# samedii/perceptor

Hardware: AMD Instinct MI355X
Metric: denoising steps/sec (UNet+CLIP-grad) at 512x512 batch 8 (higher is better)
Workload: dtype bf16

## Files before the change

perceptor_amd/csrc/attn.hip:

```cpp
#include "common.h"
#include "../../include/perceptor_hip.h"

namespace {

__device__ __forceinline__ int64_t tfrag(int bh, int ntb, int tb, int ks, int db, int lhi, int l31) {
  return ((((((int64_t)bh * ntb + tb) * 2 + ks) * 2 + db) * 2 + lhi) * 32 + l31) * 8;
}

__device__ __forceinline__ int64_t rfrag(int bh, int ntb, int tb, int kk, int lhi, int l31) {
  return ((((((int64_t)bh * ntb + tb) * 4 + kk) * 2 + lhi) * 32 + l31) * 8);
}

template <typename T_>
__global__ __launch_bounds__(256) void qkv_split_kernel(const u16* __restrict__ qkv, u16* __restrict__ q,
                                                        u16* __restrict__ k, u16* __restrict__ vt, int T, int Tp,
                                                        int heads, int order) {
  __shared__ u16 sv[32][72];
  const int tid = threadIdx.x, t0 = blockIdx.x * 32, bh = blockIdx.y;
  const int n = bh / heads, h = bh - n * heads;
  const int C = heads * 64;
  const int qoff = order == 0 ? h * 192 : h * 64;
  const int koff = order == 0 ? h * 192 + 64 : C + h * 64;
  const int voff = order == 0 ? h * 192 + 128 : 2 * C + h * 64;
  const int row = tid >> 3, ch = tid & 7;
// ... 162 lines not shown
                                                          int T, int Tp, int heads) {
  __shared__ u16 s[32][72];
  const int tid = threadIdx.x, t0 = blockIdx.x * 32, bh = blockIdx.y;
  const int n = bh / heads, h = bh - n * heads, C = heads * 64;
  const int row = tid >> 3, ch = tid & 7, t = t0 + row;
  uint4 val = make_uint4(0, 0, 0, 0), ov = val;
  if (t < T) {
    val = *(const uint4*)(dout + ((int64_t)n * T + t) * C + h * 64 + ch * 8);
    ov = *(const uint4*)(o + ((int64_t)n * T + t) * C + h * 64 + ch * 8);
  }
  *(uint4*)(d_o + rfrag(bh, Tp >> 5, blockIdx.x, ch >> 1, ch & 1, row)) = val;
  *(uint4*)(&s[row][ch * 8]) = val;
  float a[8], b[8], p = 0.f;
  unpack8<T_>(val, a); unpack8<T_>(ov, b);
#pragma unroll
  for (int e = 0; e < 8; ++e) p += a[e] * b[e];
  p += __shfl_xor(p, 1); p += __shfl_xor(p, 2); p += __shfl_xor(p, 4);
  if (ch == 0) delta[(int64_t)bh * Tp + t] = p;
  __syncthreads();
  const int d = tid >> 2, tc = tid & 3, fks = tc >> 1, flhi = tc & 1;
  u16 e[8];
#pragma unroll
  for (int j = 0; j < 8; ++j) e[j] = s[16 * fks + 4 * flhi + (j & 3) + 8 * (j >> 2)][d];
  *(uint4*)(d_ot + tfrag(bh, Tp >> 5, blockIdx.x, fks, d >> 5, flhi, d & 31)) =
      make_uint4(e[0] | (e[1] << 16), e[2] | (e[3] << 16), e[4] | (e[5] << 16), e[6] | (e[7] << 16));
}

template <typename T_>
__global__ __launch_bounds__(64) void vit_attn_fwd_kernel(const u16* __restrict__ q, const u16* __restrict__ k, const u16* __restrict__ vt,
                                                          u16* __restrict__ out, float* __restrict__ lse, int T, int Tp, int heads, float scale) {
  const int lane = threadIdx.x, l31 = lane & 31, lhi = lane >> 5;
  int bx, bh;
  head_xcd_remap(bx, bh);
  const int t0 = bx * 32;
  const int ntb = Tp >> 5;
  uint4 qf[4];
#pragma unroll
  for (int kk = 0; kk < 4; ++kk) qf[kk] = *(const uint4*)(q + rfrag(bh, ntb, bx, kk, lhi, l31));
  f32x16 o0, o1;
#pragma unroll
  for (int r = 0; r < 16; ++r) { o0[r] = 0.f; o1[r] = 0.f; }
  float m_run = -1e30f, l_run = 0.f;
  struct Tile { uint4 k[4], vt[2][2]; };
  auto load_tile = [&](int sb, Tile& f) {
#pragma unroll
    for (int kk = 0; kk < 4; ++kk) f.k[kk] = *(const uint4*)(k + rfrag(bh, ntb, sb, kk, lhi, l31));
#pragma unroll
    for (int ks = 0; ks < 2; ++ks)
#pragma unroll
      for (int db = 0; db < 2; ++db) f.vt[ks][db] = *(const uint4*)(vt + tfrag(bh, ntb, sb, ks, db, lhi, l31));
  };
  auto compute = [&](const Tile& f, int s0) {
    f32x16 sacc;
#pragma unroll
    for (int r = 0; r < 16; ++r) sacc[r] = 0.f;
#pragma unroll
    for (int kk = 0; kk < 4; ++kk) sacc = T_::mfma32(f.k[kk], qf[kk], sacc);
    float mx = -1e30f;
#pragma unroll
    for (int r = 0; r < 16; ++r) {
      const int s = s0 + (r & 3) + 8 * (r >> 2) + 4 * lhi;
      const float v = s < T ? sacc[r] * scale : -1e30f;
      sacc[r] = v; mx = fmaxf(mx, v);
    }
    mx = fmaxf(mx, __shfl_xor(mx, 32));
    const float m_new = fmaxf(m_run, mx), alpha = __expf(m_run - m_new);
    float rs = 0.f;
#pragma unroll
    for (int r = 0; r < 16; ++r) { const float p = __expf(sacc[r] - m_new); sacc[r] = p; rs += p; }
    rs += __shfl_xor(rs, 32);
    l_run = l_run * alpha + rs; m_run = m_new;
#pragma unroll
    for (int r = 0; r < 16; ++r) { o0[r] *= alpha; o1[r] *= alpha; }
#pragma unroll
    for (int ks = 0; ks < 2; ++ks) {
      float pf[8];
#pragma unroll
      for (int j = 0; j < 8; ++j) pf[j] = sacc[8 * ks + j];
      const uint4 pfrag = pack8<T_>(pf);
      o0 = T_::mfma32(f.vt[ks][0], pfrag, o0);
      o1 = T_::mfma32(f.vt[ks][1], pfrag, o1);
    }
  };
  Tile ta, tb_;
  load_tile(0, ta);
  for (int sb = 0; sb < ntb; sb += 2) {
    load_tile(sb + 1 < ntb ? sb + 1 : sb, tb_);
    __builtin_amdgcn_sched_barrier(0);
    compute(ta, sb * 32);
    __builtin_amdgcn_sched_barrier(0);
    if (sb + 1 < ntb) {
      load_tile(sb + 2 < ntb ? sb + 2 : sb + 1, ta);
      __builtin_amdgcn_sched_barrier(0);
      compute(tb_, (sb + 1) * 32);
      __builtin_amdgcn_sched_barrier(0);
    }
  }
  const int t = t0 + l31;
  if (lhi == 0) lse[(int64_t)bh * Tp + t] = t < T ? m_run + __logf(l_run) : 0.f;
  if (t < T) {
    const float inv = 1.f / l_run;
    const int n = bh / heads, h = bh - n * heads;
    u16* ob = out + ((int64_t)n * T + t) * (heads * 64) + h * 64 + 4 * lhi;
#pragma unroll
    for (int g = 0; g < 4; ++g) {
      *(uint2*)(ob + 8 * g) = pack4<T_>(o0[4 * g] * inv, o0[4 * g + 1] * inv, o0[4 * g + 2] * inv, o0[4 * g + 3] * inv);
      *(uint2*)(ob + 32 + 8 * g) = pack4<T_>(o1[4 * g] * inv, o1[4 * g + 1] * inv, o1[4 * g + 2] * inv, o1[4 * g + 3] * inv);
    }
  }
}

template <typename T_>
__device__ __forceinline__ void vit_attn_dq_body(const u16* __restrict__ q, const u16* __restrict__ k, const u16* __restrict__ v,
                                                 const u16* __restrict__ kt, const u16* __restrict__ d_o,
                                                 const float* __restrict__ lse, const float* __restrict__ delta,
                                                 u16* __restrict__ dqkv, int T, int Tp, int heads, float scale, int bx, int bh) {
  const int lane = threadIdx.x, l31 = lane & 31, lhi = lane >> 5;
  const int t0 = bx * 32;
  const int64_t rb = (int64_t)bh * Tp;
  uint4 qf[4], dof[4];
#pragma unroll
  for (int kk = 0; kk < 4; ++kk) {
    qf[kk] = *(const uint4*)(q + rfrag(bh, Tp >> 5, bx, kk, lhi, l31));
    dof[kk] = *(const uint4*)(d_o + rfrag(bh, Tp >> 5, bx, kk, lhi, l31));
  }
  const float my_lse = lse[rb + t0 + l31], my_delta = delta[rb + t0 + l31];
  f32x16 g0, g1;
#pragma unroll
  for (int r = 0; r < 16; ++r) { g0[r] = 0.f; g1[r] = 0.f; }
  struct Tile { uint4 k[4], v[4], kt[2][2]; };
  const int ntb = Tp >> 5;
  auto load_tile = [&](int sb, Tile& f) {
#pragma unroll
    for (int kk = 0; kk < 4; ++kk) {
      f.k[kk] = *(const uint4*)(k + rfrag(bh, ntb, sb, kk, lhi, l31));
      f.v[kk] = *(const uint4*)(v + rfrag(bh, ntb, sb, kk, lhi, l31));
    }
#pragma unroll
    for (int ks = 0; ks < 2; ++ks)
#pragma unroll
      for (int db = 0; db < 2; ++db) f.kt[ks][db] = *(const uint4*)(kt + tfrag(bh, ntb, sb, ks, db, lhi, l31));
  };
  auto compute = [&](const Tile& f, int s0) {
    f32x16 sacc, dp;
#pragma unroll
    for (int r = 0; r < 16; ++r) { sacc[r] = 0.f; dp[r] = 0.f; }
#pragma unroll
    for (int kk = 0; kk < 4; ++kk) {
      sacc = T_::mfma32(f.k[kk], qf[kk], sacc);
      dp = T_::mfma32(f.v[kk], dof[kk], dp);
    }
#pragma unroll
    for (int r = 0; r < 16; ++r) {
      const int s = s0 + (r & 3) + 8 * (r >> 2) + 4 * lhi;
      const float p = s < T ? __expf(sacc[r] * scale - my_lse) : 0.f;
      sacc[r] = p * (dp[r] - my_delta) * scale;
    }
#pragma unroll
    for (int ks = 0; ks < 2; ++ks) {
      float g[8];
#pragma unroll
      for (int j = 0; j < 8; ++j) g[j] = sacc[8 * ks + j];
      const uint4 dsf = pack8<T_>(g);
      g0 = T_::mfma32(f.kt[ks][0], dsf, g0);
      g1 = T_::mfma32(f.kt[ks][1], dsf, g1);
    }
  };
  Tile ta, tb_;
  load_tile(0, ta);
  for (int sb = 0; sb < ntb; sb += 2) {
    load_tile(sb + 1 < ntb ? sb + 1 : sb, tb_);
    __builtin_amdgcn_sched_barrier(0);
    compute(ta, sb * 32);
    __builtin_amdgcn_sched_barrier(0);
    if (sb + 1 < ntb) {
      load_tile(sb + 2 < ntb ? sb + 2 : sb + 1, ta);
      __builtin_amdgcn_sched_barrier(0);
      compute(tb_, (sb + 1) * 32);
      __builtin_amdgcn_sched_barrier(0);
    }
  }
  const int t = t0 + l31;
  if (t < T) {
    const int n = bh / heads, h = bh - n * heads, C = heads * 64;
    u16* ob = dqkv + ((int64_t)n * T + t) * 3 * C + h * 64 + 4 * lhi;
#pragma unroll
    for (int g = 0; g < 4; ++g) {
      *(uint2*)(ob + 8 * g) = pack4<T_>(g0[4 * g], g0[4 * g + 1], g0[4 * g + 2], g0[4 * g + 3]);
      *(uint2*)(ob + 32 + 8 * g) = pack4<T_>(g1[4 * g], g1[4 * g + 1], g1[4 * g + 2], g1[4 * g + 3]);
    }
  }
}

template <typename T_>
__device__ __forceinline__ void vit_attn_dkdv_body(const u16* __restrict__ q, const u16* __restrict__ k, const u16* __restrict__ v,
                                                   const u16* __restrict__ qt, const u16* __restrict__ d_o, const u16* __restrict__ d_ot,
                                                   const float* __restrict__ lse, const float* __restrict__ delta,
                                                   u16* __restrict__ dqkv, int T, int Tp, int heads, float scale, int bx, int bh) {
  const int lane = threadIdx.x, l31 = lane & 31, lhi = lane >> 5;
  const int s0 = bx * 32;
  const int64_t rb = (int64_t)bh * Tp;
  uint4 kf[4], vf[4];
#pragma unroll
  for (int kk = 0; kk < 4; ++kk) {
    kf[kk] = *(const uint4*)(k + rfrag(bh, Tp >> 5, bx, kk, lhi, l31));
    vf[kk] = *(const uint4*)(v + rfrag(bh, Tp >> 5, bx, kk, lhi, l31));
  }
  const bool key_ok = s0 + l31 < T;
  f32x16 dk0, dk1, dv0, dv1;
#pragma unroll
  for (int r = 0; r < 16; ++r) { dk0[r] = 0.f; dk1[r] = 0.f; dv0[r] = 0.f; dv1[r] = 0.f; }
  struct Tile { uint4 q[4], dO[4], dot[2][2], qt[2][2]; float ls[16], dl[16]; };
  const int ntb = Tp >> 5;
  auto load_tile = [&](int tb, Tile& f) {
#pragma unroll
    for (int kk = 0; kk < 4; ++kk) {
      f.q[kk] = *(const uint4*)(q + rfrag(bh, ntb, tb, kk, lhi, l31));
      f.dO[kk] = *(const uint4*)(d_o + rfrag(bh, ntb, tb, kk, lhi, l31));
    }
#pragma unroll
    for (int ks = 0; ks < 2; ++ks)
#pragma unroll
      for (int db = 0; db < 2; ++db) {
        const int64_t fo = tfrag(bh, ntb, tb, ks, db, lhi, l31);
        f.dot[ks][db] = *(const uint4*)(d_ot + fo); f.qt[ks][db] = *(const uint4*)(qt + fo);
      }
#pragma unroll
    for (int r = 0; r < 16; ++r) {
      const int t = tb * 32 + (r & 3) + 8 * (r >> 2) + 4 * lhi;
      f.ls[r] = lse[rb + t]; f.dl[r] = delta[rb + t];
    }
  };
  auto compute = [&](const Tile& f, int t0) {
    f32x16 sacc, dp;
#pragma unroll
    for (int r = 0; r < 16; ++r) { sacc[r] = 0.f; dp[r] = 0.f; }
#pragma unroll
    for (int kk = 0; kk < 4; ++kk) {
      sacc = T_::mfma32(f.q[kk], kf[kk], sacc);
      dp = T_::mfma32(f.dO[kk], vf[kk], dp);
    }
    float pf[16];
#pragma unroll
    for (int r = 0; r < 16; ++r) {
      const int t = t0 + (r & 3) + 8 * (r >> 2) + 4 * lhi;
      const float p = (key_ok && t < T) ? __expf(sacc[r] * scale - f.ls[r]) : 0.f;
      pf[r] = p;
      sacc[r] = p * (dp[r] - f.dl[r]) * scale;
    }
#pragma unroll
    for (int ks = 0; ks < 2; ++ks) {
      const uint4 pfrag = pack8<T_>(pf + 8 * ks);
      float g[8];
#pragma unroll
      for (int j = 0; j < 8; ++j) g[j] = sacc[8 * ks + j];
      const uint4 dsf = pack8<T_>(g);
      dv0 = T_::mfma32(f.dot[ks][0], pfrag, dv0); dk0 = T_::mfma32(f.qt[ks][0], dsf, dk0);
      dv1 = T_::mfma32(f.dot[ks][1], pfrag, dv1); dk1 = T_::mfma32(f.qt[ks][1], dsf, dk1);
    }
  };
  Tile ta, tb_;
  load_tile(0, ta);
  for (int tb = 0; tb < ntb; tb += 2) {
    load_tile(tb + 1 < ntb ? tb + 1 : tb, tb_);
    __builtin_amdgcn_sched_barrier(0);
    compute(ta, tb * 32);
    __builtin_amdgcn_sched_barrier(0);
    if (tb + 1 < ntb) {
      load_tile(tb + 2 < ntb ? tb + 2 : tb + 1, ta);
      __builtin_amdgcn_sched_barrier(0);
      compute(tb_, (tb + 1) * 32);
      __builtin_amdgcn_sched_barrier(0);
    }
  }
  const int s = s0 + l31;
  if (s < T) {
    const int n = bh / heads, h = bh - n * heads, C = heads * 64;
    u16* okp = dqkv + ((int64_t)n * T + s) * 3 * C + C + h * 64 + 4 * lhi;
    u16* ovp = okp + C;
#pragma unroll
    for (int g = 0; g < 4; ++g) {
      *(uint2*)(okp + 8 * g) = pack4<T_>(dk0[4 * g], dk0[4 * g + 1], dk0[4 * g + 2], dk0[4 * g + 3]);
      *(uint2*)(okp + 32 + 8 * g) = pack4<T_>(dk1[4 * g], dk1[4 * g + 1], dk1[4 * g + 2], dk1[4 * g + 3]);
      *(uint2*)(ovp + 8 * g) = pack4<T_>(dv0[4 * g], dv0[4 * g + 1], dv0[4 * g + 2], dv0[4 * g + 3]);
      *(uint2*)(ovp + 32 + 8 * g) = pack4<T_>(dv1[4 * g], dv1[4 * g + 1], dv1[4 * g + 2], dv1[4 * g + 3]);
    }
  }
}

template <typename T_>
__global__ __launch_bounds__(64) void vit_attn_bwd_kernel(const u16* __restrict__ q, const u16* __restrict__ k, const u16* __restrict__ v,
                                                          const u16* __restrict__ qt, const u16* __restrict__ kt,
                                                          const u16* __restrict__ d_o, const u16* __restrict__ d_ot,
                                                          const float* __restrict__ lse, const float* __restrict__ delta,
                                                          u16* __restrict__ dqkv, int T, int Tp, int heads, float scale) {
  int bx, bh;
  head_xcd_remap(bx, bh);
  if (blockIdx.z == 0) vit_attn_dkdv_body<T_>(q, k, v, qt, d_o, d_ot, lse, delta, dqkv, T, Tp, heads, scale, bx, bh);
  else vit_attn_dq_body<T_>(q, k, v, kt, d_o, lse, delta, dqkv, T, Tp, heads, scale, bx, bh);
}

}

#define VIT_BY_DTYPE(KERN, G, B, ...)                                                             \
  do {                                                                                            \
    if (dtype == PMI_DT_BF16) hipLaunchKernelGGL(KERN<BF16>, G, B, 0, (hipStream_t)s, __VA_ARGS__); \
    else hipLaunchKernelGGL(KERN<F16>, G, B, 0, (hipStream_t)s, __VA_ARGS__);                     \
  } while (0)

extern "C" int pmi_vit_attn_fwd(const void* qkv, void* ws16, float* lse, void* out, int N, int T, int heads, float scale, int dtype,
                                pmi_stream_t s) {
  if (!qkv || !ws16 || !lse || !out || N <= 0 || T <= 0 || heads <= 0) return PMI_ERR_ARG;
  const int Tp = (T + 31) / 32 * 32;
  const int64_t blk = (int64_t)N * heads * Tp * 64;
  u16* w = (u16*)ws16;
  dim3 g(Tp / 32, N * heads);
  VIT_BY_DTYPE(vit_qkv_split_kernel, g, dim3(256), (const u16*)qkv, w, w + blk, w + 2 * blk, w + 3 * blk, w + 4 * blk, w + 5 * blk, T, Tp, heads);
  PMI_CHECK_LAUNCH();
  VIT_BY_DTYPE(vit_attn_fwd_kernel, g, dim3(64), w, w + blk, w + 5 * blk, (u16*)out, lse, T, Tp, heads, scale);
  PMI_CHECK_LAUNCH();
  return PMI_OK;
}

extern "C" int pmi_vit_attn_bwd(const void* ws16, const float* lse, const void* o, const void* dout, void* ws16b, float* delta,
                                void* dqkv, int N, int T, int heads, float scale, int dtype, pmi_stream_t s) {
  if (!ws16 || !lse || !o || !dout || !ws16b || !delta || !dqkv || N <= 0 || T <= 0 || heads <= 0) return PMI_ERR_ARG;
  const int Tp = (T + 31) / 32 * 32;
  const int64_t blk = (int64_t)N * heads * Tp * 64;
  const u16* w = (const u16*)ws16;
  u16* wb = (u16*)ws16b;
  dim3 g(Tp / 32, N * heads);
  VIT_BY_DTYPE(vit_do_prep_kernel, g, dim3(256), (const u16*)dout, (const u16*)o, wb, wb + blk, delta, T, Tp, heads);
  PMI_CHECK_LAUNCH();
  dim3 g2(Tp / 32, N * heads, 2);
  VIT_BY_DTYPE(vit_attn_bwd_kernel, g2, dim3(64), w, w + blk, w + 2 * blk, w + 3 * blk, w + 4 * blk, wb, wb + blk, lse, delta, (u16*)dqkv, T, Tp,
               heads, scale);
  PMI_CHECK_LAUNCH();
  return PMI_OK;
}
```

perceptor_amd/csrc/igemm.hip:

```cpp
#include <cstdio>
#include <cstdlib>
#include "common.h"
#include "epilogue.h"
#include "../../include/perceptor_hip.h"

namespace {

constexpr int BM = 128, BN = 128, BK = 64;
constexpr int TILE_BYTES = 128 * 128;
constexpr int STAGE_BYTES = 2 * TILE_BYTES;

__device__ __forceinline__ int lds_off(int row, int chunk) { return row * 128 + ((chunk ^ ((row >> 1) & 7)) << 4); }

template <typename T, bool CONV, bool KFAST, bool PHASED = false>
__global__ __launch_bounds__(256, 2) void igemm_kernel(const pmi_igemm_args a) {
  static_assert(!PHASED || CONV, "the phased geometry is a convolution");
  __shared__ __attribute__((aligned(16))) char smem[2 * STAGE_BYTES];

  const int tid = threadIdx.x, lane = tid & 63, wid = tid >> 6;
  const int wr = wid >> 1, wc = wid & 1;
#ifdef PMI_STAMPS
#define GSTAMP(k) do { if (tid == 0 && a.reserved == 77 && a.splitk <= 1) ((long long*)a.ws)[(int64_t)blockIdx.x * 8 + (k)] = (long long)wall_clock64(); } while (0)
#else
#define GSTAMP(k) do {} while (0)
// ... 267 lines not shown
#pragma unroll
    for (int e = 0; e < 16; ++e) cs[e] = 0.f;
#pragma unroll
    for (int t = 0; t < 8; ++t) {
      const int m = m0 + wr * 64 + 8 * t + rp;
      uint4 v = *(const uint4*)(stg + (8 * t + rp) * SROW + r8 * 16);
      if (a.R || a.stats) {
        float f[8];
        unpack8<T>(v, f);
        if (a.R) {
          float r[8];
          unpack8<T>(rres[t], r);
#pragma unroll
          for (int e = 0; e < 8; ++e) f[e] += r[e];
          v = pack8<T>(f);
        }
        if (m < a.M) {
#pragma unroll
          for (int e = 0; e < 8; ++e) { cs[e] += f[e]; cs[8 + e] += f[e] * f[e]; }
        }
      }
      if (nok && m < Mr) *(uint4*)((u16*)a.D + offD + orow(m) * a.ldd + n0 + cl0) = v;
    }
    if (a.stats) {
      float b8[8], b4[4], b2[2];
      const bool h3 = lane & 8, h4 = lane & 16, h5 = lane & 32;
#pragma unroll
      for (int k = 0; k < 8; ++k) { const float mine = h3 ? cs[k + 8] : cs[k], other = h3 ? cs[k] : cs[k + 8]; b8[k] = mine + __shfl_xor(other, 8); }
#pragma unroll
      for (int k = 0; k < 4; ++k) { const float mine = h4 ? b8[k + 4] : b8[k], other = h4 ? b8[k] : b8[k + 4]; b4[k] = mine + __shfl_xor(other, 16); }
#pragma unroll
      for (int k = 0; k < 2; ++k) { const float mine = h5 ? b4[k + 2] : b4[k], other = h5 ? b4[k] : b4[k + 2]; b2[k] = mine + __shfl_xor(other, 32); }
      const int e0 = (h4 ? 4 : 0) + (h5 ? 2 : 0);
      float* const slot = stat + wr * 2 * BN;
      slot[2 * (cl0 + e0) + (h3 ? 1 : 0)] = b2[0];
      slot[2 * (cl0 + e0 + 1) + (h3 ? 1 : 0)] = b2[1];
    }
  } else {
  int64_t rrow[2];
  const float* nbp[2];
  int mrow[2];
#pragma unroll
  for (int i = 0; i < 2; ++i) {
    const int m = m0 + wr * 64 + i * 32 + l31;
    mrow[i] = m;
    rrow[i] = (int64_t)m * a.ldr;
    if (a.R && a.res_up && m < a.M) {
      const int hw = a.H * a.W;
      const int img = m / hw, rem = m - img * hw;
      const int y = rem / a.W, x = rem - y * a.W;
      rrow[i] = ((int64_t)(img * (a.H >> 1) + (y >> 1)) * (a.W >> 1) + (x >> 1)) * a.ldr;
    }
    nbp[i] = (a.nbias && m < a.M) ? a.nbias + (int64_t)(m / a.hw) * (a.ldnb ? a.ldnb : a.N) : nullptr;
  }
#pragma unroll
  for (int j = 0; j < 2; ++j) {
    float ssum[16], ssq[16];
#pragma unroll
    for (int r = 0; r < 16; ++r) { ssum[r] = 0.f; ssq[r] = 0.f; }
    float4 rv[2][4], bv[4], nbv[2][4];
#pragma unroll
    for (int g = 0; g < 4; ++g) {
      const int n = n0 + wc * 64 + j * 32 + 4 * lhi + 8 * g;
      bv[g] = make_float4(0.f, 0.f, 0.f, 0.f);
      if (a.bias && n < a.N) bv[g] = *(const float4*)(a.bias + n);
#pragma unroll
      for (int i = 0; i < 2; ++i) {
        nbv[i][g] = make_float4(0.f, 0.f, 0.f, 0.f);
        if (nbp[i] && n < a.N) nbv[i][g] = *(const float4*)(nbp[i] + n);
      }
    }
    if (a.R) {
#pragma unroll
      for (int i = 0; i < 2; ++i)
#pragma unroll
        for (int g = 0; g < 4; ++g) {
          const int n = n0 + wc * 64 + j * 32 + 4 * lhi + 8 * g;
          rv[i][g] = make_float4(0.f, 0.f, 0.f, 0.f);
          if (mrow[i] >= a.M || n >= a.N) continue;
          if (a.res_f32) {
            rv[i][g] = *(const float4*)((const float*)a.R + offR + rrow[i] + n);
          } else if (a.split_out) {
            const int po = split_off(n, a.split_out);
            const uint2 rh = *(const uint2*)((const u16*)a.R + offR + rrow[i] + po);
            const uint2 rl = *(const uint2*)((const u16*)a.R + offR + rrow[i] + po + a.split_out);
            rv[i][g].x = __builtin_bit_cast(float, rh.x); rv[i][g].y = __builtin_bit_cast(float, rh.y);
            rv[i][g].z = __builtin_bit_cast(float, rl.x); rv[i][g].w = __builtin_bit_cast(float, rl.y);
          } else {
            const uint2 r = *(const uint2*)((const u16*)a.R + offR + rrow[i] + n);
            rv[i][g].x = __builtin_bit_cast(float, r.x); rv[i][g].y = __builtin_bit_cast(float, r.y);
          }
        }
    }
#pragma unroll
    for (int i = 0; i < 2; ++i) {
      const int m = mrow[i];
      if (m >= Mr) continue;
      const int64_t mo = orow(m);
#pragma unroll
      for (int g = 0; g < 4; ++g) {
        const int n = n0 + wc * 64 + j * 32 + 4 * lhi + 8 * g;
        if (n >= a.N) continue;
        float v[4];
#pragma unroll
        for (int e = 0; e < 4; ++e) v[e] = acc[i][j][4 * g + e] * a.alpha;
        v[0] += bv[g].x + nbv[i][g].x; v[1] += bv[g].y + nbv[i][g].y; v[2] += bv[g].z + nbv[i][g].z; v[3] += bv[g].w + nbv[i][g].w;
        if (a.act != PMI_ACT_NONE) act_apply_n<4>(v, a.act);
        if (a.R) {
          if (a.res_f32) {
            v[0] += rv[i][g].x; v[1] += rv[i][g].y; v[2] += rv[i][g].z; v[3] += rv[i][g].w;
          } else {
            const uint32_t r0 = __builtin_bit_cast(uint32_t, rv[i][g].x), r1 = __builtin_bit_cast(uint32_t, rv[i][g].y);
            v[0] += T::to_f((u16)(r0 & 0xffff)); v[1] += T::to_f((u16)(r0 >> 16));
            v[2] += T::to_f((u16)(r1 & 0xffff)); v[3] += T::to_f((u16)(r1 >> 16));
            if (a.split_out) {
              const uint32_t l0 = __builtin_bit_cast(uint32_t, rv[i][g].z), l1 = __builtin_bit_cast(uint32_t, rv[i][g].w);
              v[0] += T::to_f((u16)(l0 & 0xffff)); v[1] += T::to_f((u16)(l0 >> 16));
              v[2] += T::to_f((u16)(l1 & 0xffff)); v[3] += T::to_f((u16)(l1 >> 16));
            }
          }
        }
        if (a.split_out) {
          const int64_t o = offD + (int64_t)m * a.ldd + split_off(n, a.split_out);
          const uint2 hi = pack4<T>(v[0], v[1], v[2], v[3]);
          const float l0 = v[0] - T::to_f((u16)(hi.x & 0xffff)), l1 = v[1] - T::to_f((u16)(hi.x >> 16));
          const float l2 = v[2] - T::to_f((u16)(hi.y & 0xffff)), l3 = v[3] - T::to_f((u16)(hi.y >> 16));
          *(uint2*)((u16*)a.D + o) = hi;
          *(uint2*)((u16*)a.D + o + a.split_out) = pack4<T>(l0, l1, l2, l3);
        } else {
        const int64_t o = offD + mo * a.ldd + n;
        if (a.out_f32) *(float4*)((float*)a.D + o) = make_float4(v[0], v[1], v[2], v[3]);
        else *(uint2*)((u16*)a.D + o) = pack4<T>(v[0], v[1], v[2], v[3]);
        }
#pragma unroll
        for (int e = 0; e < 4; ++e) { ssum[4 * g + e] += v[e]; ssq[4 * g + e] += v[e] * v[e]; }
      }
    }
    if (a.stats) stats_block_to_lds(ssum, ssq, stat + wr * 2 * BN, wc * 64 + j * 32, lane);
  }
  }
  if (a.stats) {
    __syncthreads();
    const int img = m0 / a.hw, prow = (m0 - img * a.hw) / BM;
    float* o = a.stats + ((int64_t)(img * a.stats_p + prow) * a.N + n0) * 2;
    for (int c = tid; c < 2 * BN; c += 256)
      if (n0 + (c >> 1) < a.N) o[c] = stat[c] + stat[2 * BN + c];
  }
#ifdef PMI_STAMPS
  __syncthreads();
  GSTAMP(3);
#endif
}

template <typename T>
__global__ __launch_bounds__(256) void splitk_reduce_kernel(const pmi_igemm_args a) {
  const int n4 = a.N >> 2;
  const int64_t total = (int64_t)a.M * n4;
  const float* ws = (const float*)a.ws;
  for (int64_t i = (int64_t)blockIdx.x * 256 + threadIdx.x; i < total; i += (int64_t)gridDim.x * 256) {
    const int m = (int)(i / n4), n = (int)(i - (int64_t)m * n4) * 4;
    float4 s = make_float4(0.f, 0.f, 0.f, 0.f);
    for (int z = 0; z < a.splitk; ++z) {
      const float4 p = *(const float4*)(ws + ((int64_t)z * a.M + m) * a.N + n);
      s.x += p.x; s.y += p.y; s.z += p.z; s.w += p.w;
    }
    float v[4] = {s.x * a.alpha, s.y * a.alpha, s.z * a.alpha, s.w * a.alpha};
    if (a.bias) { const float4 b = *(const float4*)(a.bias + n); v[0] += b.x; v[1] += b.y; v[2] += b.z; v[3] += b.w; }
    if (a.nbias) {
      const float4 b = *(const float4*)(a.nbias + (int64_t)(m / a.hw) * (a.ldnb ? a.ldnb : a.N) + n);
      v[0] += b.x; v[1] += b.y; v[2] += b.z; v[3] += b.w;
    }
    if (a.act != PMI_ACT_NONE) act_apply_n<4>(v, a.act);
    if (a.R) {
      int64_t rrow = (int64_t)m * a.ldr;
      if (a.res_up) {
        const int hw = a.H * a.W;
        const int img = m / hw, rem = m - img * hw;
        const int y = rem / a.W, x = rem - y * a.W;
        rrow = ((int64_t)(img * (a.H >> 1) + (y >> 1)) * (a.W >> 1) + (x >> 1)) * a.ldr;
      }
      if (a.res_f32) {
        const float4 r = *(const float4*)((const float*)a.R + rrow + n);
        v[0] += r.x; v[1] += r.y; v[2] += r.z; v[3] += r.w;
      } else {
        const int po = a.split_out ? split_off(n, a.split_out) : n;
        const uint2 r = *(const uint2*)((const u16*)a.R + rrow + po);
        v[0] += T::to_f((u16)(r.x & 0xffff)); v[1] += T::to_f((u16)(r.x >> 16));
        v[2] += T::to_f((u16)(r.y & 0xffff)); v[3] += T::to_f((u16)(r.y >> 16));
        if (a.split_out) {
          const uint2 l = *(const uint2*)((const u16*)a.R + rrow + po + a.split_out);
          v[0] += T::to_f((u16)(l.x & 0xffff)); v[1] += T::to_f((u16)(l.x >> 16));
          v[2] += T::to_f((u16)(l.y & 0xffff)); v[3] += T::to_f((u16)(l.y >> 16));
        }
      }
    }
    if (a.split_out) {
      const int64_t o = (int64_t)m * a.ldd + split_off(n, a.split_out);
      const uint2 hi = pack4<T>(v[0], v[1], v[2], v[3]);
      const float l0 = v[0] - T::to_f((u16)(hi.x & 0xffff)), l1 = v[1] - T::to_f((u16)(hi.x >> 16));
      const float l2 = v[2] - T::to_f((u16)(hi.y & 0xffff)), l3 = v[3] - T::to_f((u16)(hi.y >> 16));
      *(uint2*)((u16*)a.D + o) = hi;
      *(uint2*)((u16*)a.D + o + a.split_out) = pack4<T>(l0, l1, l2, l3);
      continue;
    }
    const int64_t o = (int64_t)m * a.ldd + n;
    if (a.out_f32) *(float4*)((float*)a.D + o) = make_float4(v[0], v[1], v[2], v[3]);
    else *(uint2*)((u16*)a.D + o) = pack4<T>(v[0], v[1], v[2], v[3]);
  }
}

template <typename T>
int launch(const pmi_igemm_args& a, hipStream_t s) {
  const bool phased = a.up == 2;
  const int tiles = (((phased ? a.M / 4 : a.M) + BM - 1) / BM) * ((a.N + BN - 1) / BN);
  const dim3 grid(tiles, phased ? 4 : 1, a.batch > 1 ? a.batch : (a.splitk > 1 ? a.splitk : 1)), block(256);
  const bool conv = a.taps != 1 || a.up || a.stride == 2;
  const int Cin = a.C0 + a.C1;
  const bool kfast = (Cin % BK == 0) && (a.C0 % BK == 0);
  if (phased) {
    if (kfast) hipLaunchKernelGGL((igemm_kernel<T, true, true, true>), grid, block, 0, s, a);
    else hipLaunchKernelGGL((igemm_kernel<T, true, false, true>), grid, block, 0, s, a);
  } else if (conv) {
    if (kfast) hipLaunchKernelGGL((igemm_kernel<T, true, true>), grid, block, 0, s, a);
    else hipLaunchKernelGGL((igemm_kernel<T, true, false>), grid, block, 0, s, a);
  } else {
    if (kfast) hipLaunchKernelGGL((igemm_kernel<T, false, true>), grid, block, 0, s, a);
    else hipLaunchKernelGGL((igemm_kernel<T, false, false>), grid, block, 0, s, a);
  }
  PMI_CHECK_LAUNCH();
  if (a.splitk > 1) {
    const int64_t work = (int64_t)a.M * (a.N / 4);
    const int blocks = (int)((work + 255) / 256 > 4096 ? 4096 : (work + 255) / 256);
    hipLaunchKernelGGL(splitk_reduce_kernel<T>, dim3(blocks), dim3(256), 0, s, a);
    PMI_CHECK_LAUNCH();
  }
  return PMI_OK;
}

}

extern "C" int pmi_conv3x3_halo_config(const pmi_igemm_args* a);
int pmi_conv3x3_halo_launch(const pmi_igemm_args* a, int cfg, void* stream);
int pmi_conv3x3_wd_launch(const pmi_igemm_args* a, int cfg, void* stream);
int pmi_conv3x3_up_wd_launch(const pmi_igemm_args* a, void* stream);
extern "C" int pmi_gemm_wd_eligible(const pmi_igemm_args* a);
int pmi_gemm_wd_tile_rows(const pmi_igemm_args* a, int splitk);
int pmi_gemm_wd_launch(const pmi_igemm_args* a, void* stream);
void pmi_conv3x3_allow_wd(int v);
void pmi_conv3x3_wd_mf16(int v);
void pmi_conv3x3_wd128(int v);
void pmi_conv3x3_force_config(int cfg);
void pmi_conv3x3_prefer_256(int v);
static int g_allow_halo = 1;
static int g_wd_max_split = 8;
int pmi_conv3x3_wd_splitk(const pmi_igemm_args* a, int cfg);
extern "C" int pmi_igemm_splitk(const pmi_igemm_args* a) {
  if (a->batch > 1 || (a->N & 3) || a->up == 2) return 1;
  if (g_allow_halo) {
    const int halo = pmi_conv3x3_halo_config(a);
    if (halo >= 0) return pmi_conv3x3_wd_splitk(a, halo);
  }
  if (a->act == PMI_ACT_GEGLU) return 1;
  if (a->A1 && a->taps == 1 && pmi_gemm_wd_eligible(a)) return 1;
  if (pmi_gemm_wd_eligible(a)) {
    const int nch = (a->K + 127) / 128;
    int best = 1;
    long best_cost = -1;
    for (int s = 1; s <= g_wd_max_split && nch / s >= 4; s *= 2) {
      const int rows = pmi_gemm_wd_tile_rows(a, s);
      const long wgs = (long)((a->M + rows - 1) / rows) * (a->N < 256 ? 1 : (a->N + 255) / 256) * s;
      const long cost = ((wgs + 255) / 256) * rows * (nch / s + 6) + (s > 1 ? 8L * 144 : 0);
      if (best_cost < 0 || cost < best_cost) { best_cost = cost; best = s; }
    }
    return best;
  }
  const int tiles = ((a->M + BM - 1) / BM) * ((a->N + BN - 1) / BN);
  const int nk = (a->K + BK - 1) / BK;
  if (tiles >= 384 || nk < 16) return 1;
  int s = 512 / tiles;
  if (s > nk / 8) s = nk / 8;
  if (s > 16) s = 16;
  return s < 2 ? 1 : s;
}

int pmi_igemm_halo_allowed(void) { return g_allow_halo; }

extern "C" int pmi_igemm_stats_rows(const pmi_igemm_args* a) {
  if (a->batch > 1 || a->splitk > 1 || a->up == 2) return 0;
  const int halo = g_allow_halo ? pmi_conv3x3_halo_config(a) : -1;
  if (a->split_out) return halo >= 6 ? (a->H / 8) * (a->W / 32) : 0;
  if (halo == 3) return 0;
  if (halo >= 0) return (a->H / (halo == 1 ? 16 : 8)) * (a->W / 32);
  if (a->hw > 0 && (a->hw % BM) == 0 && (a->M % a->hw) == 0) return a->hw / BM;
  return 0;
}

void pmi_attn_flash_qt(int v);
void pmi_attn_flash_kv_chunks(int v);
void pmi_conv3x3_wd_splitk_enable(int v);
void pmi_gemm_wd_few_wgs(int v);
void pmi_conv3x3_wd_smallc(int v);
void pmi_conv3x3_up_phase(int v);
void pmi_conv3x3_skip_enable(int v);

extern "C" int pmi_set_option(int key, int value) {
  if (key == 0) { const int old = g_allow_halo; g_allow_halo = value; return old; }
  if (key == 1) { pmi_conv3x3_force_config(value); return 0; }
  if (key == 2) { pmi_conv3x3_prefer_256(value); return 0; }
  if (key == 6) { pmi_conv3x3_allow_wd(value); return 0; }
  if (key == 7) { pmi_conv3x3_wd_mf16(value); return 0; }
  if (key == 8) { pmi_conv3x3_wd128(value); return 0; }
  if (key == 9) { pmi_attn_flash_qt(value); return 0; }
  if (key == 10) { pmi_conv3x3_wd_splitk_enable(value); return 0; }
  if (key == 11) { g_wd_max_split = value; return 0; }
  if (key == 12) { pmi_gemm_wd_few_wgs(value); return 0; }
  if (key == 13) { pmi_conv3x3_wd_smallc(value); return 0; }
  if (key == 14) { pmi_attn_flash_kv_chunks(value); return 0; }
  if (key == 15) { pmi_conv3x3_up_phase(value); return 0; }
  if (key == 16) { pmi_conv3x3_skip_enable(value); return 0; }
  return PMI_ERR_ARG;
}

static int bad_arg(int line) {
  if (getenv("PMI_DEBUG")) fprintf(stderr, "pmi_igemm: argument check at igemm.hip:%d failed\n", line);
  return PMI_ERR_ARG;
}

extern "C" int pmi_igemm(const pmi_igemm_args* a, pmi_stream_t stream) {
  if (!a || !a->A0 || !a->B || !a->D) return bad_arg(__LINE__);
  if (a->M <= 0 || a->N <= 0 || a->K <= 0) return bad_arg(__LINE__);
  if ((a->K & 7) || (a->C0 & 7) || (a->C1 & 7)) return bad_arg(__LINE__);
  if ((a->N & 3) && (a->bias || a->nbias || a->R || a->ldd < ((a->N + 3) & ~3))) return bad_arg(__LINE__);
  if ((a->lda0 & 7) || (a->ldb & 7) || (a->ldd & 3)) return bad_arg(__LINE__);
  if (a->C1 > 0 && (!a->A1 || (a->lda1 & 7))) return bad_arg(__LINE__);
  if (a->taps != 1 && a->taps != 9 && a->taps != 16) return bad_arg(__LINE__);
  if (a->taps == 16 && (a->stride != 2 || a->up || a->res_up || a->Hin != 2 * a->H || a->Win != 2 * a->W)) return bad_arg(__LINE__);
  if (a->stride != 1 && a->stride != 2) return bad_arg(__LINE__);
  if (a->up == 2 && (a->taps != 9 || a->stride != 2 || a->res_up || a->A1 || a->C1 || a->R || a->nbias || a->stats || a->splitk > 1 || a->batch > 1 ||
                     a->split_out || a->split_in || a->pro_a || a->D2 || a->aux || a->dtype == PMI_DT_F16X2 || (a->M & 3))) return bad_arg(__LINE__);
  if (a->K != a->taps * (a->C0 + a->C1)) return bad_arg(__LINE__);
  if (a->R && (a->ldr & 3)) return bad_arg(__LINE__);
  if (a->split_out && ((a->split_out & 7) || a->split_out > 32 || a->out_f32 || (a->N % a->split_out) || a->batch > 1)) return bad_arg(__LINE__);
  if ((unsigned)a->split_in > 2u) return bad_arg(__LINE__);
  if (a->split_in == 2 && !a->split_out) return bad_arg(__LINE__);
  if (a->nbias && a->hw <= 0) return bad_arg(__LINE__);
  const bool conv = a->taps != 1 || a->up || a->stride == 2;
  if (a->res_up && ((a->H & 1) || (a->W & 1))) return bad_arg(__LINE__);
  if ((conv || a->res_up) && (a->H <= 0 || a->W <= 0 || a->Hin <= 0 || a->Win <= 0 || a->M % (a->H * a->W))) return bad_arg(__LINE__);
  if (a->up && (a->H != 2 * a->Hin || a->W != 2 * a->Win)) return bad_arg(__LINE__);
  if (a->batch > 1 && a->batch_inner <= 0) return bad_arg(__LINE__);
  const int halo = g_allow_halo ? pmi_conv3x3_halo_config(a) : -1;
  if (a->pro_a && (!a->pro_b || halo < 0)) return PMI_ERR_ARG;
  if ((a->split_in == 2 || ((a->split_in || a->split_out) && a->pro_a) || (a->split_out && a->R && a->res_f32)) && halo < 6) return bad_arg(__LINE__);
  if (a->stats && a->stats_p != pmi_igemm_stats_rows(a)) return PMI_ERR_ARG;
  if (a->splitk > 1 && (!a->ws || a->batch > 1 || (halo >= 0 && a->splitk != pmi_conv3x3_wd_splitk(a, halo)) || (a->N & 3) || a->stats)) return PMI_ERR_ARG;
  if (a->act == PMI_ACT_GEGLU && !pmi_gemm_wd_eligible(a)) return bad_arg(__LINE__);
  if ((a->D2 || a->aux) && !pmi_gemm_wd_eligible(a)) return bad_arg(__LINE__);
  if (pmi_gemm_wd_eligible(a) && !((a->nbias || a->res_up) && a->splitk <= 1)) {
    const int rc = pmi_gemm_wd_launch(a, stream);
    if (rc != PMI_OK || a->splitk <= 1 || a->reserved3 == 1) return rc;
    hipStream_t s = (hipStream_t)stream;
    const int64_t work = (int64_t)a->M * (a->N / 4);
    const int blocks = (int)((work + 255) / 256 > 4096 ? 4096 : (work + 255) / 256);
    if (a->dtype == PMI_DT_BF16) hipLaunchKernelGGL(splitk_reduce_kernel<BF16>, dim3(blocks), dim3(256), 0, s, *a);
    else hipLaunchKernelGGL(splitk_reduce_kernel<F16>, dim3(blocks), dim3(256), 0, s, *a);
    PMI_CHECK_LAUNCH();
    return PMI_OK;
  }
  if (halo == 9) return pmi_conv3x3_up_wd_launch(a, stream);
  if (halo >= 4) {
    const int rc = pmi_conv3x3_wd_launch(a, halo, stream);
    if (rc != PMI_OK || a->splitk <= 1) return rc;
    hipStream_t s = (hipStream_t)stream;
    const int64_t work = (int64_t)a->M * (a->N / 4);
    const int blocks = (int)((work + 255) / 256 > 4096 ? 4096 : (work + 255) / 256);
    if (a->dtype == PMI_DT_BF16) hipLaunchKernelGGL(splitk_reduce_kernel<BF16>, dim3(blocks), dim3(256), 0, s, *a);
    else hipLaunchKernelGGL(splitk_reduce_kernel<F16>, dim3(blocks), dim3(256), 0, s, *a);
    PMI_CHECK_LAUNCH();
    return PMI_OK;
  }
  if (halo >= 0) return pmi_conv3x3_halo_launch(a, halo, stream);
  hipStream_t s = (hipStream_t)stream;
  return a->dtype == PMI_DT_BF16 ? launch<BF16>(*a, s) : launch<F16>(*a, s);
}

extern "C" int pmi_abi_version(void) { return 1; }
```

Before: 26.78.

## Add whole-sequence LDS-resident ViT attention kernels for short sequences

Adds forward and backward ViT attention kernels for sequences up to 288 tokens (CLIP ViT, 257 tokens). Each workgroup holds the whole K/V (forward) or Q/K/V/dO (backward) of one head in LDS. The forward kernel fuses the qkv split into the attention pass. The backward kernel fuses the dO·O delta prep and uses only two workgroups per head, one computing dK/dV and one computing dQ. This removes separate split and prep launches and repeated global reads of K/V, but needs up to about 147 KB of dynamic LDS and leaves few workgroups per head, which may underfill the GPU.

```diff
diff --git a/perceptor_amd/csrc/attn.hip b/perceptor_amd/csrc/attn.hip
--- a/perceptor_amd/csrc/attn.hip
+++ b/perceptor_amd/csrc/attn.hip
@@ -488,11 +488,344 @@
 
 }
 
+namespace {
+
+constexpr int VL_MAX_TP = 288;
+constexpr int VL_FWD_QT = 5;
+constexpr int VL_BWD_WAVES = 9;
+
+typedef short vl_s4 __attribute__((ext_vector_type(4)));
+
+__device__ __forceinline__ int vl_off(int t, int ch) {
+  return (t >> 5) * 4096 + ch * 512 + (((t & 31) ^ ((ch & 3) << 2)) << 4);
+}
+
+struct VlLane {
+  int row0, row1;
+  int tr;
+  __device__ __forceinline__ VlLane(int lane) {
+    const int l31 = lane & 31, lhi = lane >> 5;
+    row0 = lhi * 512 + ((l31 ^ (lhi << 2)) << 4);
+    row1 = lhi * 512 + ((l31 ^ ((2 + lhi) << 2)) << 4);
+    const int q = (lane >> 2) & 3, p = lane & 3, k = 2 * ((lane >> 4) & 1) + (p >> 1);
+    tr = k * 512 + ((((4 * lhi) ^ (4 * k)) + q) << 4) + 8 * (p & 1);
+  }
+};
+
+__device__ __forceinline__ uint4 vl_row_frag(const unsigned char* img, const VlLane& L, int tb, int kk) {
+  return *(const uint4*)(img + tb * 4096 + kk * 1024 + ((kk & 1) ? L.row1 : L.row0));
+}
+__device__ __forceinline__ uint4 vl_tr_frag(const unsigned char* img, const VlLane& L, int tb, int ks, int db) {
+  typedef __attribute__((address_space(3))) vl_s4* lds_s4;
+  const unsigned char* p = img + tb * 4096 + db * 2048 + ks * 256;
+  const vl_s4 a = __builtin_amdgcn_ds_read_tr16_b64_v4i16((lds_s4)(p + L.tr));
+  const vl_s4 b = __builtin_amdgcn_ds_read_tr16_b64_v4i16((lds_s4)(p + (L.tr ^ 128)));
+  const uint2 ua = __builtin_bit_cast(uint2, a), ub = __builtin_bit_cast(uint2, b);
+  return make_uint4(ua.x, ua.y, ub.x, ub.y);
+}
+
+template <typename T_>
+__global__ __launch_bounds__(VL_FWD_QT * 64) void vit_attn_fwd_lds_kernel(const u16* __restrict__ qkv, u16* __restrict__ wq, u16* __restrict__ wk,
+                                                                            u16* __restrict__ wv, u16* __restrict__ out, float* __restrict__ lse,
+                                                                            int T, int Tp, int heads, float scale) {
+  extern __shared__ __align__(16) unsigned char vl_smem[];
+  unsigned char* ki = vl_smem;
+  unsigned char* vi = vl_smem + Tp * 128;
+  const int tid = threadIdx.x, lane = tid & 63, wave = tid >> 6, l31 = lane & 31, lhi = lane >> 5;
+  int part, bh;
+  head_xcd_remap(part, bh);
+  const int n = bh / heads, h = bh - n * heads, C = heads * 64, ntb = Tp >> 5;
+  const u16* src = qkv + (int64_t)n * T * 3 * C + h * 64;
+  constexpr int NT = VL_FWD_QT * 64, IT = (VL_MAX_TP * 8 + NT - 1) / NT;
+  uint4 kr[IT], vr[IT];
+#pragma unroll
+  for (int i = 0; i < IT; ++i) {
+    const int e = i * NT + tid, t = (e >> 6) * 8 + (e & 7), ch = (e >> 3) & 7;
+    const u16* p = src + (int64_t)(t < T ? t : T - 1) * 3 * C + ch * 8;
+    kr[i] = *(const uint4*)(p + C); vr[i] = *(const uint4*)(p + 2 * C);
+    if (t >= T) { kr[i] = make_uint4(0, 0, 0, 0); vr[i] = kr[i]; }
+  }
+  const int bx = part * VL_FWD_QT + wave;
+  const bool active = bx < ntb;
+  const int t0 = bx * 32;
+  uint4 qf[4];
+#pragma unroll
+  for (int kk = 0; kk < 4; ++kk) {
+    const int t = t0 + l31;
+    qf[kk] = *(const uint4*)(src + (int64_t)(t < T ? t : T - 1) * 3 * C + kk * 16 + lhi * 8);
+    if (t >= T) qf[kk] = make_uint4(0, 0, 0, 0);
+  }
+#pragma unroll
+  for (int i = 0; i < IT; ++i) {
+    const int e = i * NT + tid, t = (e >> 6) * 8 + (e & 7), ch = (e >> 3) & 7;
+    if (e < Tp * 8) {
+      const int o = vl_off(t, ch);
+      *(uint4*)(ki + o) = kr[i]; *(uint4*)(vi + o) = vr[i];
+      const int64_t g = rfrag(bh, ntb, t >> 5, ch >> 1, ch & 1, t & 31);
+      if (part == 0) *(uint4*)(wk + g) = kr[i];
+      if (part == (int)gridDim.x - 1) *(uint4*)(wv + g) = vr[i];
+    }
+  }
+  if (active) {
+#pragma unroll
+    for (int kk = 0; kk < 4; ++kk) *(uint4*)(wq + rfrag(bh, ntb, bx, kk, lhi, l31)) = qf[kk];
+  }
+  __syncthreads();
+  if (!active) return;
+  const VlLane L(lane);
+  f32x16 o0, o1;
+#pragma unroll
+  for (int r = 0; r < 16; ++r) { o0[r] = 0.f; o1[r] = 0.f; }
+  float m_run = -1e30f, l_run = 0.f;
+  for (int sb = 0; sb < ntb; ++sb) {
+    const int s0 = sb * 32;
+    f32x16 sacc;
+#pragma unroll
+    for (int r = 0; r < 16; ++r) sacc[r] = 0.f;
+#pragma unroll
+    for (int kk = 0; kk < 4; ++kk) sacc = T_::mfma32(vl_row_frag(ki, L, sb, kk), qf[kk], sacc);
+    uint4 vt[2][2];
+#pragma unroll
+    for (int k2 = 0; k2 < 2; ++k2)
+#pragma unroll
+      for (int db = 0; db < 2; ++db) vt[k2][db] = vl_tr_frag(vi, L, sb, k2, db);
+    float mx = -1e30f;
+#pragma unroll
+    for (int r = 0; r < 16; ++r) {
+      const int s = s0 + (r & 3) + 8 * (r >> 2) + 4 * lhi;
+      const float v = s < T ? sacc[r] * scale : -1e30f;
+      sacc[r] = v; mx = fmaxf(mx, v);
+    }
+    mx = fmaxf(mx, __shfl_xor(mx, 32));
+    const float m_new = fmaxf(m_run, mx), alpha = __expf(m_run - m_new);
+    float rs = 0.f;
+#pragma unroll
+    for (int r = 0; r < 16; ++r) { const float p = __expf(sacc[r] - m_new); sacc[r] = p; rs += p; }
+    rs += __shfl_xor(rs, 32);
+    l_run = l_run * alpha + rs; m_run = m_new;
+#pragma unroll
+    for (int r = 0; r < 16; ++r) { o0[r] *= alpha; o1[r] *= alpha; }
+#pragma unroll
+    for (int k2 = 0; k2 < 2; ++k2) {
+      float pf[8];
+#pragma unroll
+      for (int j = 0; j < 8; ++j) pf[j] = sacc[8 * k2 + j];
+      const uint4 pfrag = pack8<T_>(pf);
+      o0 = T_::mfma32(vt[k2][0], pfrag, o0);
+      o1 = T_::mfma32(vt[k2][1], pfrag, o1);
+    }
+  }
+  const int t = t0 + l31;
+  if (lhi == 0) lse[(int64_t)bh * Tp + t] = t < T ? m_run + __logf(l_run) : 0.f;
+  if (t < T) {
+    const float inv = 1.f / l_run;
+    u16* ob = out + ((int64_t)n * T + t) * C + h * 64 + 4 * lhi;
+#pragma unroll
+    for (int g = 0; g < 4; ++g) {
+      *(uint2*)(ob + 8 * g) = pack4<T_>(o0[4 * g] * inv, o0[4 * g + 1] * inv, o0[4 * g + 2] * inv, o0[4 * g + 3] * inv);
+      *(uint2*)(ob + 32 + 8 * g) = pack4<T_>(o1[4 * g] * inv, o1[4 * g + 1] * inv, o1[4 * g + 2] * inv, o1[4 * g + 3] * inv);
+    }
+  }
+}
+
+template <typename T_>
+__global__ __launch_bounds__(VL_BWD_WAVES * 64) void vit_attn_bwd_lds_kernel(const u16* __restrict__ wq, const u16* __restrict__ wk,
+                                                                            const u16* __restrict__ wv, const u16* __restrict__ dout,
+                                                                            const u16* __restrict__ o, const float* __restrict__ lse,
+                                                                            u16* __restrict__ dqkv, int T, int Tp, int heads, float scale) {
+  extern __shared__ __align__(16) unsigned char vl_smem[];
+  unsigned char* qi = vl_smem;
+  unsigned char* ki = qi + Tp * 128;
+  unsigned char* vi = ki + Tp * 128;
+  unsigned char* di = vi + Tp * 128;
+  float* ls = (float*)(di + Tp * 128);
+  float* dl = ls + Tp;
+  const int tid = threadIdx.x, lane = tid & 63, wave = tid >> 6, l31 = lane & 31, lhi = lane >> 5;
+  int role, bh;
+  head_xcd_remap(role, bh);
+  const int n = bh / heads, h = bh - n * heads, C = heads * 64, ntb = Tp >> 5;
+  constexpr int NT = VL_BWD_WAVES * 64, IT = VL_MAX_TP * 8 / NT;
+  static_assert(IT * NT == VL_MAX_TP * 8, "items per thread");
+  {
+    const uint4* gq = (const uint4*)(wq + (int64_t)bh * Tp * 64);
+    const uint4* gk = (const uint4*)(wk + (int64_t)bh * Tp * 64);
+    const uint4* gv = (const uint4*)(wv + (int64_t)bh * Tp * 64);
+    uint4 a[IT], b[IT], c[IT];
+#pragma unroll
+    for (int i = 0; i < IT; ++i) {
+      const int e = i * NT + tid, ec = e < Tp * 8 ? e : Tp * 8 - 1;
+      a[i] = gq[ec]; b[i] = gk[ec]; c[i] = gv[ec];
+    }
+#pragma unroll
+    for (int i = 0; i < IT; ++i) {
+      const int e = i * NT + tid;
+      if (e < Tp * 8) {
+        const int off = vl_off((e >> 8) * 32 + (e & 31), (e >> 5) & 7);
+        *(uint4*)(qi + off) = a[i]; *(uint4*)(ki + off) = b[i]; *(uint4*)(vi + off) = c[i];
+      }
+    }
+  }
+  {
+    const int64_t base = (int64_t)n * T * C + h * 64;
+    uint4 a[IT], b[IT];
+#pragma unroll
+    for (int i = 0; i < IT; ++i) {
+      const int e = i * NT + tid, t = (e >> 6) * 8 + (e & 7), ch = (e >> 3) & 7;
+      const int64_t g = base + (int64_t)(t < T ? t : T - 1) * C + ch * 8;
+      a[i] = *(const uint4*)(dout + g); b[i] = *(const uint4*)(o + g);
+      if (t >= T) { a[i] = make_uint4(0, 0, 0, 0); b[i] = a[i]; }
+    }
+#pragma unroll
+    for (int i = 0; i < IT; ++i) {
+      const int e = i * NT + tid, t = (e >> 6) * 8 + (e & 7), ch = (e >> 3) & 7;
+      if (e < Tp * 8) {
+        *(uint4*)(di + vl_off(t, ch)) = a[i];
+        float x[8], y[8], p = 0.f;
+        unpack8<T_>(a[i], x); unpack8<T_>(b[i], y);
+#pragma unroll
+        for (int j = 0; j < 8; ++j) p += x[j] * y[j];
+        p += __shfl_xor(p, 8); p += __shfl_xor(p, 16); p += __shfl_xor(p, 32);
+        if (ch == 0) dl[t] = p;
+      }
+    }
+    for (int t = tid; t < Tp; t += NT) ls[t] = lse[(int64_t)bh * Tp + t];
+  }
+  __syncthreads();
+  if (wave >= ntb) return;
+  const VlLane L(lane);
+  const int bx = wave;
+  if (role == 0) {
+    const bool key_ok = bx * 32 + l31 < T;
+    f32x16 dk0, dk1, dv0, dv1;
+#pragma unroll
+    for (int r = 0; r < 16; ++r) { dk0[r] = 0.f; dk1[r] = 0.f; dv0[r] = 0.f; dv1[r] = 0.f; }
+    for (int tb = 0; tb < ntb; ++tb) {
+      const int t0 = tb * 32;
+      int bxo = bx;
+      asm volatile("" : "+v"(bxo));
+      f32x16 sacc, dp;
+#pragma unroll
+      for (int r = 0; r < 16; ++r) { sacc[r] = 0.f; dp[r] = 0.f; }
+#pragma unroll
+      for (int kk = 0; kk < 4; ++kk) {
+        sacc = T_::mfma32(vl_row_frag(qi, L, tb, kk), vl_row_frag(ki, L, bxo, kk), sacc);
+        dp = T_::mfma32(vl_row_frag(di, L, tb, kk), vl_row_frag(vi, L, bxo, kk), dp);
+      }
+      float pf[16];
+#pragma unroll
+      for (int g = 0; g < 4; ++g) {
+        const float4 l4 = *(const float4*)(ls + t0 + 8 * g + 4 * lhi), d4 = *(const float4*)(dl + t0 + 8 * g + 4 * lhi);
+        const float lv[4] = {l4.x, l4.y, l4.z, l4.w}, dv[4] = {d4.x, d4.y, d4.z, d4.w};
+#pragma unroll
+        for (int j = 0; j < 4; ++j) {
+          const int r = 4 * g + j, t = t0 + 8 * g + 4 * lhi + j;
+          const float p = (key_ok && t < T) ? __expf(sacc[r] * scale - lv[j]) : 0.f;
+          pf[r] = p;
+          sacc[r] = p * (dp[r] - dv[j]) * scale;
+        }
+      }
+#pragma unroll
+      for (int ks = 0; ks < 2; ++ks) {
+        const uint4 pfrag = pack8<T_>(pf + 8 * ks);
+        float g[8];
+#pragma unroll
+        for (int j = 0; j < 8; ++j) g[j] = sacc[8 * ks + j];
+        const uint4 dsf = pack8<T_>(g);
+        dv0 = T_::mfma32(vl_tr_frag(di, L, tb, ks, 0), pfrag, dv0); dk0 = T_::mfma32(vl_tr_frag(qi, L, tb, ks, 0), dsf, dk0);
+        dv1 = T_::mfma32(vl_tr_frag(di, L, tb, ks, 1), pfrag, dv1); dk1 = T_::mfma32(vl_tr_frag(qi, L, tb, ks, 1), dsf, dk1);
+      }
+    }
+    const int s = bx * 32 + l31;
+    if (s < T) {
+      u16* okp = dqkv + ((int64_t)n * T + s) * 3 * C + C + h * 64 + 4 * lhi;
+      u16* ovp = okp + C;
+#pragma unroll
+      for (int g = 0; g < 4; ++g) {
+        *(uint2*)(okp + 8 * g) = pack4<T_>(dk0[4 * g], dk0[4 * g + 1], dk0[4 * g + 2], dk0[4 * g + 3]);
+        *(uint2*)(okp + 32 + 8 * g) = pack4<T_>(dk1[4 * g], dk1[4 * g + 1], dk1[4 * g + 2], dk1[4 * g + 3]);
+        *(uint2*)(ovp + 8 * g) = pack4<T_>(dv0[4 * g], dv0[4 * g + 1], dv0[4 * g + 2], dv0[4 * g + 3]);
+        *(uint2*)(ovp + 32 + 8 * g) = pack4<T_>(dv1[4 * g], dv1[4 * g + 1], dv1[4 * g + 2], dv1[4 * g + 3]);
+      }
+    }
+  } else {
+    uint4 qf[4], dof[4];
+#pragma unroll
+    for (int kk = 0; kk < 4; ++kk) { qf[kk] = vl_row_frag(qi, L, bx, kk); dof[kk] = vl_row_frag(di, L, bx, kk); }
+    const float my_lse = ls[bx * 32 + l31], my_delta = dl[bx * 32 + l31];
+    f32x16 g0, g1;
+#pragma unroll
+    for (int r = 0; r < 16; ++r) { g0[r] = 0.f; g1[r] = 0.f; }
+    for (int sb = 0; sb < ntb; ++sb) {
+      const int s0 = sb * 32;
+      f32x16 sacc, dp;
+#pragma unroll
+      for (int r = 0; r < 16; ++r) { sacc[r] = 0.f; dp[r] = 0.f; }
+#pragma unroll
+      for (int kk = 0; kk < 4; ++kk) {
+        sacc = T_::mfma32(vl_row_frag(ki, L, sb, kk), qf[kk], sacc);
+        dp = T_::mfma32(vl_row_frag(vi, L, sb, kk), dof[kk], dp);
+      }
+#pragma unroll
+      for (int r = 0; r < 16; ++r) {
+        const int s = s0 + (r & 3) + 8 * (r >> 2) + 4 * lhi;
+        const float p = s < T ? __expf(sacc[r] * scale - my_lse) : 0.f;
+        sacc[r] = p * (dp[r] - my_delta) * scale;
+      }
+#pragma unroll
+      for (int ks = 0; ks < 2; ++ks) {
+        float g[8];
+#pragma unroll
+        for (int j = 0; j < 8; ++j) g[j] = sacc[8 * ks + j];
+        const uint4 dsf = pack8<T_>(g);
+        g0 = T_::mfma32(vl_tr_frag(ki, L, sb, ks, 0), dsf, g0);
+        g1 = T_::mfma32(vl_tr_frag(ki, L, sb, ks, 1), dsf, g1);
+      }
+    }
+    const int t = bx * 32 + l31;
+    if (t < T) {
+      u16* ob = dqkv + ((int64_t)n * T + t) * 3 * C + h * 64 + 4 * lhi;
+#pragma unroll
+      for (int g = 0; g < 4; ++g) {
+        *(uint2*)(ob + 8 * g) = pack4<T_>(g0[4 * g], g0[4 * g + 1], g0[4 * g + 2], g0[4 * g + 3]);
+        *(uint2*)(ob + 32 + 8 * g) = pack4<T_>(g1[4 * g], g1[4 * g + 1], g1[4 * g + 2], g1[4 * g + 3]);
+      }
+    }
+  }
+}
+
+}
+
+static int g_vit_lds = 1;
+void pmi_vit_attn_lds(int v) { g_vit_lds = v; }
+
+static bool vit_lds_route(int T, int dtype) {
+  return g_vit_lds && (T + 31) / 32 * 32 <= VL_MAX_TP && (dtype == PMI_DT_BF16 || dtype == PMI_DT_F16);
+}
+
+template <typename K>
+static bool vl_allow_lds(K kern, int bytes) {
+  static bool done[64] = {};
+  int dev = 0;
+  if (bytes <= 64 * 1024) return true;
+  if (hipGetDevice(&dev) != hipSuccess || dev < 0 || dev >= 64) return false;
+  if (!done[dev]) done[dev] = hipFuncSetAttribute((const void*)kern, hipFuncAttributeMaxDynamicSharedMemorySize, 160 * 1024) == hipSuccess;
+  return done[dev];
+}
+
 #define VIT_BY_DTYPE(KERN, G, B, ...)                                                             \
   do {                                                                                            \
     if (dtype == PMI_DT_BF16) hipLaunchKernelGGL(KERN<BF16>, G, B, 0, (hipStream_t)s, __VA_ARGS__); \
     else hipLaunchKernelGGL(KERN<F16>, G, B, 0, (hipStream_t)s, __VA_ARGS__);                     \
   } while (0)
+
+template <typename K, typename... A>
+static bool vl_launch(K kern, dim3 g, int threads, int bytes, pmi_stream_t s, A... args) {
+  if (!vl_allow_lds(kern, bytes)) return false;
+  hipLaunchKernelGGL(kern, g, dim3(threads), bytes, (hipStream_t)s, args...);
+  return true;
+}
+#define VIT_LDS_LAUNCH(KERN, G, B, BYTES, ...) \
+  (dtype == PMI_DT_BF16 ? vl_launch(KERN<BF16>, G, B, BYTES, s, __VA_ARGS__) : vl_launch(KERN<F16>, G, B, BYTES, s, __VA_ARGS__))
 
 extern "C" int pmi_vit_attn_fwd(const void* qkv, void* ws16, float* lse, void* out, int N, int T, int heads, float scale, int dtype,
                                 pmi_stream_t s) {
@@ -500,6 +833,13 @@
   const int Tp = (T + 31) / 32 * 32;
   const int64_t blk = (int64_t)N * heads * Tp * 64;
   u16* w = (u16*)ws16;
+  if (vit_lds_route(T, dtype)) {
+    const bool ok = VIT_LDS_LAUNCH(vit_attn_fwd_lds_kernel, dim3((Tp / 32 + VL_FWD_QT - 1) / VL_FWD_QT, N * heads), VL_FWD_QT * 64, 2 * Tp * 128, (const u16*)qkv,
+                                   w, w + blk, w + 2 * blk, (u16*)out, lse, T, Tp, heads, scale);
+    if (!ok) return PMI_ERR_LAUNCH;
+    PMI_CHECK_LAUNCH();
+    return PMI_OK;
+  }
   dim3 g(Tp / 32, N * heads);
   VIT_BY_DTYPE(vit_qkv_split_kernel, g, dim3(256), (const u16*)qkv, w, w + blk, w + 2 * blk, w + 3 * blk, w + 4 * blk, w + 5 * blk, T, Tp, heads);
   PMI_CHECK_LAUNCH();
@@ -515,6 +855,14 @@
   const int64_t blk = (int64_t)N * heads * Tp * 64;
   const u16* w = (const u16*)ws16;
   u16* wb = (u16*)ws16b;
+  if (vit_lds_route(T, dtype)) {
+    const int bytes = 4 * Tp * 128 + 2 * Tp * 4;
+    const bool ok = VIT_LDS_LAUNCH(vit_attn_bwd_lds_kernel, dim3(2, N * heads), VL_BWD_WAVES * 64, bytes, w, w + blk, w + 2 * blk, (const u16*)dout, (const u16*)o,
+                                   lse, (u16*)dqkv, T, Tp, heads, scale);
+    if (!ok) return PMI_ERR_LAUNCH;
+    PMI_CHECK_LAUNCH();
+    return PMI_OK;
+  }
   dim3 g(Tp / 32, N * heads);
   VIT_BY_DTYPE(vit_do_prep_kernel, g, dim3(256), (const u16*)dout, (const u16*)o, wb, wb + blk, delta, T, Tp, heads);
   PMI_CHECK_LAUNCH();
diff --git a/perceptor_amd/csrc/igemm.hip b/perceptor_amd/csrc/igemm.hip
--- a/perceptor_amd/csrc/igemm.hip
+++ b/perceptor_amd/csrc/igemm.hip
@@ -593,6 +593,7 @@
 void pmi_conv3x3_wd_smallc(int v);
 void pmi_conv3x3_up_phase(int v);
 void pmi_conv3x3_skip_enable(int v);
+void pmi_vit_attn_lds(int v);
 
 extern "C" int pmi_set_option(int key, int value) {
   if (key == 0) { const int old = g_allow_halo; g_allow_halo = value; return old; }
@@ -609,6 +610,7 @@
   if (key == 14) { pmi_attn_flash_kv_chunks(value); return 0; }
   if (key == 15) { pmi_conv3x3_up_phase(value); return 0; }
   if (key == 16) { pmi_conv3x3_skip_enable(value); return 0; }
+  if (key == 17) { pmi_vit_attn_lds(value); return 0; }
   return PMI_ERR_ARG;
 }
 
```

After: 27.07 (median of 6 runs). +1.1%, better.
